# 0xC0000054/pdn-jpegxl

Hardware: AMD Instinct MI355X
Metric: megapixels/sec decode (4K lossy VarDCT) (higher is better)
Workload: dtype f32

## Files before the change

pdn_jpegxl_amd/csrc/dev_util.h:

```cpp
#pragma once
#include <stdint.h>
#include <hip/hip_fp16.h>

namespace jxlhip {

__host__ __device__ __forceinline__ int ReflectIndex(int v, int n) {
  while (v < 0 || v >= n) v = v < 0 ? -v - 1 : 2 * n - 1 - v;
  return v;
}

__device__ __forceinline__ uint32_t IntToOutSample(int32_t v, int bits, int out_bits) {
  const int32_t maxv = (int32_t)((1u << bits) - 1);
  if (bits == out_bits) return (uint32_t)min(maxv, max(0, v));
  float f = (float)v * (1.0f / (float)maxv);
  f *= out_bits == 16 ? 65535.0f : 255.0f;
  const float top = out_bits == 16 ? 65535.0f : 255.0f;
  if (!(f > 0.f)) return 0;
  if (f >= top) return (uint32_t)top;
  return (uint32_t)(f + 0.5f);
}

__device__ __forceinline__ float BitsToFloatSample(int32_t v, int bits) {
  if (bits == 32) return __int_as_float(v);
  return __half2float(__ushort_as_half((unsigned short)(v & 0xFFFF)));
}
__device__ __forceinline__ uint32_t FloatToOutBits(float f, int out_bits, int out_float) {
  if (out_float) return out_bits == 32 ? (uint32_t)__float_as_int(f) : (uint32_t)__half_as_ushort(__float2half_rn(f));
  const float top = out_bits == 16 ? 65535.0f : 255.0f;
  f *= top;
  if (!(f > 0.f)) return 0;
  if (f >= top) return (uint32_t)top;
  return (uint32_t)(f + 0.5f);
}
__device__ __forceinline__ uint32_t SampleToOutBits(int32_t v, int bits, int exp_bits, int out_bits, int out_float) {
  if (!out_float && !exp_bits) return IntToOutSample(v, bits, out_bits);
  const float f = exp_bits ? BitsToFloatSample(v, bits) : (float)v * (1.0f / (float)((1u << bits) - 1));
  return FloatToOutBits(f, out_bits, out_float);
}
__device__ __forceinline__ void StoreOutSample(uint8_t* base, size_t index, uint32_t raw, int out_bits) {
  if (out_bits == 8) base[index] = (uint8_t)raw;
  else if (out_bits == 16) ((uint16_t*)base)[index] = (uint16_t)raw;
  else ((uint32_t*)base)[index] = raw;
}

}
```

pdn_jpegxl_amd/csrc/entropy_kernels.hip:

```cpp
#include <hip/hip_runtime.h>
#include <cstdlib>
#include "dev_types.h"
#include "dev_util.h"
#include "kernels.h"

namespace jxlhip {

namespace {

__device__ const uint8_t d_order_bucket[kNumStrategies] = {0, 1, 1, 1, 2, 3, 4, 4, 5, 5, 6, 6, 1, 1, 1, 1, 1, 1, 7, 8, 8, 9, 10, 10, 11, 12, 12};
__device__ const uint8_t d_log2cx[kNumStrategies] = {0, 0, 0, 0, 1, 2, 0, 1, 0, 2, 1, 2, 0, 0, 0, 0, 0, 0, 3, 2, 3, 4, 3, 4, 5, 4, 5};
__device__ const uint8_t d_log2cy[kNumStrategies] = {0, 0, 0, 0, 1, 2, 1, 0, 2, 0, 2, 1, 0, 0, 0, 0, 0, 0, 3, 3, 2, 4, 4, 3, 5, 5, 4};
__device__ const uint8_t d_nnz_ctx[64] = {0,   0,   31,  62,  62,  93,  93,  93,  93,  123, 123, 123, 123, 152, 152, 152, 152, 152, 152, 152, 152, 180,
                                          180, 180, 180, 180, 180, 180, 180, 180, 180, 180, 180, 206, 206, 206, 206, 206, 206, 206, 206, 206, 206, 206,
                                          206, 206, 206, 206, 206, 206, 206, 206, 206, 206, 206, 206, 206, 206, 206, 206, 206, 206, 206, 206};

__device__ __forceinline__ int CeilLog2D(uint32_t x) { return x <= 1 ? 0 : 32 - __clz(x - 1); }
__device__ __forceinline__ int32_t UnpackSigned(uint32_t u) { return (int32_t)(u >> 1) ^ -(int32_t)(u & 1); }
#ifndef JXLHIP_PRIO_SERIAL
#define JXLHIP_PRIO_SERIAL 0
#endif
#if JXLHIP_PRIO_SERIAL
#define JXL_SERIAL_PRIO() __builtin_amdgcn_s_setprio(JXLHIP_PRIO_SERIAL)
#else
// ... 1147 lines not shown
          const int es = s_info[j];
          const int lcx = d_log2cx[es], lcy = d_log2cy[es], cx = 1 << lcx, cy = 1 << lcy;
          int wi = 0;
          uint32_t before = 0;
#pragma unroll
          for (int k = 1; k < 8; k++) { const bool past = pre[k] <= off; wi += past ? 1 : 0; before = past ? pre[k] : before; }
          uint32_t word = ~s_cov[y * 8 + wi];
          const int lim = min(32, bw - wi * 32);
          if (lim < 32) word &= (1u << lim) - 1;
          uint32_t rem = off - before;
          int xb = 0;
#pragma unroll
          for (int sft = 16; sft; sft >>= 1) {
            const uint32_t c = (uint32_t)__popc((word >> xb) & ((1u << sft) - 1));
            if (rem >= c) { rem -= c; xb += sft; }
          }
          const int x = wi * 32 + xb;
          const uint32_t mask = (cx == 32 ? 0xFFFFFFFFu : ((1u << cx) - 1)) << xb;
          if (off + (uint32_t)cx > nfree || x + cx > bw || y + cy > bh || xb + cx > 32 || (y & 31) + cy > 32 || (word & mask) != mask) {
            bad = true;
          } else {
            for (int iy = 1; iy < cy; iy++)
              if (atomicOr(&s_cov[(y + iy) * 8 + wi], mask) & mask) bad = true;
            s_pos[j] = x | y << 8;
          }
        }
      }
      const int n_row = __syncthreads_count(inrow);
      if (__syncthreads_or(bad || (nfree && !n_row))) { layout_bad = true; break; }
      num += (uint32_t)n_row;
    }
  }
  __threadfence_block();
  __syncthreads();
  if (s_flag || layout_bad || num != count) err |= kErrBlockLayout;
  if (tid == 0) s_count = (err & kErrBlockLayout) ? 0u : num;
  __syncthreads();
  const uint32_t placed = s_count;
  for (uint32_t i = tid; i < placed; i += 256) {
    const int x = s_pos[i] & 0xFF, y = s_pos[i] >> 8;
    const int s = s_info[i], q = 1 + s_info[count + i];
    const int lcx = d_log2cx[s], lcy = d_log2cy[s], cx = 1 << lcx, cy = 1 << lcy;
    const size_t cell = (size_t)(by0 + y) * im.w8 + bx0 + x;
    for (int iy = 0; iy < cy; iy++)
      for (int ix = 0; ix < cx; ix++) {
        const size_t cc = cell + (size_t)iy * im.w8 + ix;
        im.cellinfo[cc] = (uint32_t)s | ix << 8 | iy << 13 | lcx << 18 | lcy << 21 | 1u << 31;
        im.rawq[cc] = (uint16_t)q;
      }
  }
  if (err) SetError(im, err, 2, g);
}

__global__ __launch_bounds__(64) void hf_blocklist_kernel(const DevImage* __restrict__ imgs) {
  const DevImage& im = imgs[blockIdx.y];
  const int g = blockIdx.x;
  if (g >= im.ng || im.is_modular) return;
  const int lane = threadIdx.x;
  const int gx = g % im.xg, gy = g / im.xg;
  const int bx0 = gx * kGroupBlocks, by0 = gy * kGroupBlocks;
  const int bw = min(kGroupBlocks, im.w8 - bx0), bh = min(kGroupBlocks, im.h8 - by0);
  uint32_t* list = im.blk_list + (size_t)g * 1024;
  const int n_qf = im.n_qf;
  uint32_t total = 0;
  for (int it = 0; it < 16; it++) {
    const int idx = it * 64 + lane;
    const int bx = idx & 31, by = idx >> 5;
    bool first = false;
    uint32_t info = 0;
    if (bx < bw && by < bh) {
      info = im.cellinfo[(size_t)(by0 + by) * im.w8 + bx0 + bx];
      first = (info & 0x8003FF00u) == 0x80000000u;
    }
    const uint64_t m = __ballot(first);
    if (first) {
      const uint32_t pos = total + (uint32_t)__popcll(m & (((uint64_t)1 << lane) - 1));
      const uint32_t s = info & 0xFF, lcx = (info >> 18) & 7, lcy = (info >> 21) & 7;
      const uint32_t ord = d_order_bucket[s];
      const uint32_t rq = im.rawq[(size_t)(by0 + by) * im.w8 + bx0 + bx];
      uint32_t qf_idx = 0;
      for (int i = 0; i < n_qf; i++) qf_idx += rq > im.qf_thr[i];
      uint32_t lf_idx = 0;
      if (im.num_lf_ctx > 1) {
        const size_t cell = (size_t)(by0 + by) * im.w8 + bx0 + bx;
        uint32_t ix = 0, iy = 0, ib = 0;
        for (int i = 0; i < im.n_lf_thr[0]; i++) ix += im.lfq[0][cell] > im.lf_thr[0][i];
        for (int i = 0; i < im.n_lf_thr[1]; i++) iy += im.lfq[1][cell] > im.lf_thr[1][i];
        for (int i = 0; i < im.n_lf_thr[2]; i++) ib += im.lfq[2][cell] > im.lf_thr[2][i];
        lf_idx = (ix * (uint32_t)(im.n_lf_thr[2] + 1) + ib) * (uint32_t)(im.n_lf_thr[1] + 1) + iy;
      }
      uint32_t ctxs = 0;
      for (int ci = 0; ci < 3; ci++) {
        const int c = ci == 0 ? 1 : (ci == 1 ? 0 : 2);
        const uint32_t cprime = c < 2 ? (c ^ 1) : 2;
        ctxs |= ((uint32_t)im.block_ctx_map[((cprime * kNumOrders + ord) * (n_qf + 1) + qf_idx) * im.num_lf_ctx + lf_idx] & 31u) << (5 * ci);
      }
      list[pos] = (uint32_t)bx | (uint32_t)by << 5 | lcx << 10 | lcy << 13 | ctxs << 16;
    }
    total += (uint32_t)__popcll(m);
  }
  if (lane == 0) im.blk_count[g] = total;
}

template <bool kLds, int kRing>
__global__ __launch_bounds__(512) void hf_decode_kernel(const DevImage* imgs, const SectionTask* tasks, int lane_stride) {
  JXL_SERIAL_PRIO();
  constexpr int kTop = kRing / 2;
  constexpr int kQ = kRing / 4;
  typedef LaneBitsT<kRing, kRing / 4> Bits;
  extern __shared__ __align__(16) uint8_t smem[];
  const SectionTask task = tasks[blockIdx.x];
  const DevImage& im = imgs[task.image];
  const int per_wave = 64 / lane_stride;
  const int nslots = (task.count + 3) & ~3;
  CodeTab<kLds> tab;
  typename AS<kLds>::U8 nnz_tab;
  JXL_LDS uint8_t* nzcol;
  JXL_LDS uint32_t* ring_base;
  JXL_LDS uint32_t* descq;
  {
    JXL_LDS uint8_t* lds = (JXL_LDS uint8_t*)smem;
    size_t off = 0;
    ring_base = (JXL_LDS uint32_t*)lds; off += (size_t)nslots * kRing * 4;
    descq = (JXL_LDS uint32_t*)(lds + off); off += (size_t)nslots * 2 * kQ * 4;
    nzcol = lds + off; off += (size_t)nslots * 96;
    if constexpr (kLds) {
      off = StageCode(lds, off, im.acode, tab, threadIdx.x, blockDim.x);
      JXL_LDS uint8_t* sn = lds + off; off += 64;
      if (threadIdx.x < 64) sn[threadIdx.x] = d_nnz_ctx[threadIdx.x];
      nnz_tab = sn;
      __syncthreads();
    } else {
      GlobalCode(im.acode, tab);
      nnz_tab = d_nnz_ctx;
    }
  }
  if ((int)(threadIdx.x & 63) >= per_wave) return;
  const int si = (threadIdx.x >> 6) * per_wave + (threadIdx.x & 63);
  if (si >= task.count || si >= nslots) return;
  JXL_LDS uint8_t* const col = nzcol + si;
  const int g = im.hf_order[task.first + si];
  const int sec = im.single ? 0 : im.hf_sec_base + g;
  const uint64_t sec_bits = im.single ? im.hf_start_bits : im.sec_off[sec] * 8;
  Bits b;
  b.Init(im.cs, im.cs_size, sec_bits, ring_base + si, (uint32_t)nslots);
  const uint32_t preset = b.Read(CeilLog2D((uint32_t)im.num_presets));
  const uint32_t nbc = im.num_block_ctx;
  const uint32_t ctx_offset = preset * nbc * 495;
  uint32_t err = preset >= (uint32_t)im.num_presets ? (uint32_t)kErrBitstream : 0u;
  if (im.lz_hf) b.SetLz(im.lz_hf + ((size_t)g << 18), 18, 0);
  uint32_t state = InitAnsState(b, tab);
  const int gx = g % im.xg, gy = g / im.xg;
  const JXL_GLB uint32_t* const list = G(im.blk_list + (size_t)g * 1024);
  const uint32_t nblk = im.blk_count[g];
  JXL_LDS uint32_t* const dq = descq + si;
  constexpr uint32_t dqmask = 2u * kQ - 1;
  uint32_t bi = 0, dfilled = 0, it = 0, dpend_n = 0;
  uint32_t dpend[kQ];
#pragma unroll
  for (int i = 0; i < kQ; i++) dpend[i] = 0u;
  JXL_GLB uint32_t* const ent = G(im.centries) + (size_t)(g - im.centries_g0) * kGroupEntriesCap;
  const uint32_t ncells = (uint32_t)im.w8 * (uint32_t)im.h8;
  JXL_GLB U2* const cblk = (JXL_GLB U2*)G(im.cblk) + (size_t)(gy * kGroupBlocks) * im.w8 + (size_t)gx * kGroupBlocks;
  const uint32_t w8 = (uint32_t)im.w8;
  uint32_t epos = 0;
  uint32_t bx = 0, by = 0, lcx = 0, log2c = 0, covered = 1, size = 64, ctxs = 0, cell = 0;
  int ci = 3;
  uint32_t nzeros = 0, k = 0, prev = 0, histo = 0;
  bool want_nz = true;
#ifdef JXLHIP_PROFILE_HF
  const uint64_t pf_start = clock64();
  uint64_t pf_scalar = 0, pf_period = 0, pf_tokens = 0, pf_entries = 0, pf_periods = 0, pf_general = 0, pf_general_n = 0;
#endif
  uint32_t cfg_uni = 0;
  bool cfg_is_uni = false;
  if (per_wave == 1 && !tab.slow) {
    cfg_uni = tab.cfg[0] & 0xFFF;
    cfg_is_uni = true;
    for (uint32_t i = 1; i < tab.dc->num_clusters; i++) cfg_is_uni &= (tab.cfg[i] & 0xFFF) == cfg_uni;
    cfg_uni = (uint32_t)__builtin_amdgcn_readfirstlane((int)cfg_uni);
    cfg_is_uni = __builtin_amdgcn_readfirstlane((int)cfg_is_uni) != 0;
  }
  while (!err) {
    if ((it & (kTop - 1)) == 0) {
#ifdef JXLHIP_PROFILE_HF
      const uint64_t pf_t0 = clock64();
      pf_periods++;
#endif
      b.TopUp();
      if (dpend_n) {
#pragma unroll
        for (int i = 0; i < kQ; i++) if ((uint32_t)i < dpend_n) dq[__umul24((dfilled + i) & dqmask, nslots)] = dpend[i];
        dfilled += dpend_n;
        dpend_n = 0;
      }
      if (dfilled < min(nblk, bi + kQ)) {
        const uint32_t lim = min(nblk, bi + kQ);
        uint32_t v[kQ];
#pragma unroll
        for (int i = 0; i < kQ; i++) { v[i] = 0u; if (dfilled + i < lim) v[i] = list[dfilled + i]; }
#pragma unroll
        for (int i = 0; i < kQ; i++) if (dfilled + i < lim) dq[__umul24((dfilled + i) & dqmask, nslots)] = v[i];
        dfilled = lim;
      }
      {
        const uint32_t lim = min(nblk, bi + 2 * kQ);
        if (dfilled < lim) {
          dpend_n = min(lim - dfilled, (uint32_t)kQ);
#pragma unroll
          for (int i = 0; i < kQ; i++) { dpend[i] = 0u; if ((uint32_t)i < dpend_n) dpend[i] = list[dfilled + i]; }
        }
      }
#ifdef JXLHIP_PROFILE_HF
      pf_period += clock64() - pf_t0;
#endif
    }
    if (__all(!want_nz)) {
      if (per_wave == 1 && !tab.slow) {
#define JXL_RFL(x) ((uint32_t)__builtin_amdgcn_readfirstlane((int)(x)))
#ifdef JXLHIP_PROFILE_HF
        const uint64_t pf_t1 = clock64();
        pf_entries++;
#endif
        uint32_t s_state = JXL_RFL(state), s_nz = JXL_RFL(nzeros), s_k = JXL_RFL(k), s_prev = JXL_RFL(prev), s_epos = JXL_RFL(epos), s_it = JXL_RFL(it);
        const uint32_t s_cov = JXL_RFL(covered), s_l2 = JXL_RFL(log2c), s_size = JXL_RFL(size), s_histo = JXL_RFL(histo);
        uint64_t s_buf = ((uint64_t)JXL_RFL((uint32_t)(b.buf >> 32)) << 32) | JXL_RFL((uint32_t)b.buf);
        int s_n = (int)JXL_RFL(b.n);
        uint32_t s_rd = JXL_RFL(b.rd), s_rng = 0;
        const uint32_t la = JXL_RFL(tab.log_alpha), le = 12 - la;
        const uint32_t left = kTop - (s_it & (kTop - 1)), room = s_size > s_k ? s_size - s_k : 0u;
        const uint32_t cnt0 = min(left, room);
        uint32_t cnt = cnt0;
        uint32_t s_a = s_histo + 2 * JXL_RFL(nnz_tab[(s_nz + s_cov - 1) >> s_l2]);
        uint32_t s_cidx = 0xFFFFFFFFu, s_cl = 0;
        if (cnt) do {
          const uint32_t ks = s_k >> s_l2;
          const uint32_t fctx = min(ks - 1, min(7 + (ks >> 1), 15 + (ks >> 2)));
          const uint32_t cidx = s_a + fctx * 2 + s_prev;
          if (cidx != s_cidx) { s_cl = JXL_RFL(tab.cmap[cidx]); s_cidx = cidx; }
          const uint32_t cl = s_cl;
          const uint32_t res = s_state & 0xFFF, i = res >> le, pos = res & ((1u << le) - 1);
          const uint64_t e = tab.alias[(cl << la) | i];
          uint32_t c = cfg_uni;
          if (__builtin_expect(!cfg_is_uni, 0)) c = JXL_RFL(tab.cfg[cl]);
          const uint32_t x = JXL_RFL((uint32_t)e), y = JXL_RFL((uint32_t)(e >> 32));
          const bool gt = pos >= (x & 0xFF);
          const uint32_t sym = gt ? ((x >> 8) & 0xFF) : i;
          const uint32_t off = gt ? (y & 0xFFFF) + pos : pos;
          const uint32_t freq = gt ? ((x >> 16) ^ (y >> 16)) : (x >> 16);
          s_state = freq * (s_state >> 12) + off;
          if (s_state < 65536u) {
            if (s_n <= 32) { s_buf |= (uint64_t)JXL_RFL(b.ring[__umul24(s_rd & (kRing - 1), b.rs)]) << s_n; s_n += 32; s_rd++; }
            s_state = (s_state << 16) | ((uint32_t)s_buf & 0xFFFFu);
            s_buf >>= 16; s_n -= 16;
          }
          uint32_t u = sym;
          const uint32_t se = c & 0xF, split = 1u << se;
          if (__builtin_expect(sym >= split, 0)) {
            const uint32_t msb = (c >> 4) & 0xF, lsb = (c >> 8) & 0xF;
            const uint32_t nb = se - (msb + lsb) + ((sym - split) >> (msb + lsb)), nbr = nb > 32 ? 32 : nb;
            if (s_n <= 32) { s_buf |= (uint64_t)JXL_RFL(b.ring[__umul24(s_rd & (kRing - 1), b.rs)]) << s_n; s_n += 32; s_rd++; }
            const uint32_t bits = (uint32_t)(s_buf & (((uint64_t)1 << nbr) - 1));
            s_buf >>= nbr; s_n -= (int)nbr;
            const uint32_t low = sym & ((1u << lsb) - 1), hi = (1u << msb) | ((sym >> lsb) & ((1u << msb) - 1));
            u = (uint32_t)(((((uint64_t)hi << (nb & 63)) | bits) << lsb) | low);
          }
          cnt--;
          s_prev = 0;
          if (u) {
            const int32_t v = UnpackSigned(u);
            s_rng |= (uint32_t)(v + 0x8000);
            ent[s_epos++] = s_k | (uint32_t)v << 16;
            s_prev = 1;
            s_k++;
            if (--s_nz == 0) break;
            s_a = s_histo + 2 * JXL_RFL(nnz_tab[(s_nz + s_cov - 1) >> s_l2]);
          } else {
            s_k++;
          }
        } while (cnt);
        s_it += cnt0 - cnt;
#ifdef JXLHIP_PROFILE_HF
        pf_scalar += clock64() - pf_t1;
        pf_tokens += cnt0 - cnt;
#endif
        uint32_t s_err = s_rng > 0xFFFFu ? (uint32_t)kErrRange : 0u;
        if (s_nz != 0 && s_k >= s_size) s_err |= kErrBitstream;
#undef JXL_RFL
        state = s_state; nzeros = s_nz; k = s_k; prev = s_prev; epos = s_epos; it = s_it;
        b.buf = s_buf; b.n = s_n; b.rd = s_rd;
        err |= s_err;
        if (s_nz == 0 && !s_err) { want_nz = true; ci++; }
        continue;
      }
      for (;;) {
        const uint32_t nzl = (nzeros + covered - 1) >> log2c;
        const uint32_t ks = k >> log2c;
        const uint32_t fctx = ks < 16 ? ks - 1 : (ks < 32 ? 15 + ((ks - 16) >> 1) : 23 + ((ks - 32) >> 2));
        const uint32_t u = AnsGet(b, state, tab, histo + ((uint32_t)nnz_tab[nzl] + fctx) * 2 + prev);
        it++;
        bool leave = false;
        if (u) {
          const int32_t v = UnpackSigned(u);
          if (v != (int32_t)(int16_t)v) err |= kErrRange;
          ent[epos++] = k | (uint32_t)v << 16;
          prev = 1;
          if (--nzeros == 0) { want_nz = true; ci++; leave = true; }
        } else {
          prev = 0;
        }
        if (++k >= size && nzeros != 0) { err |= kErrBitstream; leave = true; }
        if (__any(leave) || (it & (kTop - 1)) == 0) break;
      }
      continue;
    }
#ifdef JXLHIP_PROFILE_HF
    const uint64_t pf_t2 = clock64();
    pf_general_n++;
#endif
    if (want_nz && ci >= 3) {
      if (bi >= nblk) break;
      const uint32_t d = dq[__umul24(bi & dqmask, nslots)];
      bi++;
      bx = d & 31; by = (d >> 5) & 31;
      lcx = (d >> 10) & 7;
      const uint32_t lcy = (d >> 13) & 7;
      ctxs = d >> 16;
      log2c = lcx + lcy; covered = 1u << log2c; size = covered << 6;
      cell = __umul24(by, w8) + bx;
      ci = 0;
    }
    const int c = ci == 0 ? 1 : (ci == 1 ? 0 : 2);
    uint32_t ctx;
    if (want_nz) {
      JXL_LDS uint8_t* const cc = col + __umul24(c * 32, nslots);
      uint32_t predicted;
      if (bx == 0) predicted = by == 0 ? 32u : (uint32_t)cc[0];
      else if (by == 0) predicted = cc[__umul24(bx - 1, nslots)];
      else predicted = ((uint32_t)cc[__umul24(bx, nslots)] + cc[__umul24(bx - 1, nslots)] + 1) >> 1;
      const uint32_t block_ctx = (ctxs >> (5 * ci)) & 31;
      uint32_t nzc = predicted >= 64 ? 64 : predicted;
      nzc = nzc < 8 ? nzc : 4 + nzc / 2;
      ctx = ctx_offset + nzc * nbc + block_ctx;
    } else {
      const uint32_t nzl = (nzeros + covered - 1) >> log2c;
      const uint32_t ks = k >> log2c;
      const uint32_t fctx = ks < 16 ? ks - 1 : (ks < 32 ? 15 + ((ks - 16) >> 1) : 23 + ((ks - 32) >> 2));
      ctx = histo + ((uint32_t)nnz_tab[nzl] + fctx) * 2 + prev;
    }
    const uint32_t u = AnsGet(b, state, tab, ctx);
    it++;
    if (want_nz) {
      nzeros = u;
      if (nzeros + covered > size) { err |= kErrBitstream; break; }
      const uint8_t fill = (uint8_t)((nzeros + covered - 1) >> log2c);
      JXL_LDS uint8_t* const cc = col + __umul24(c * 32 + bx, nslots);
      for (uint32_t ix = 0; ix < (1u << lcx); ix++) cc[__umul24(ix, nslots)] = fill;
      U2 rec;
      rec.x = epos; rec.y = nzeros;
      cblk[(size_t)c * ncells + cell] = rec;
      if (nzeros) {
        const uint32_t block_ctx = (ctxs >> (5 * ci)) & 31;
        histo = ctx_offset + nbc * 37 + 458 * block_ctx;
        prev = nzeros > size / 16 ? 0 : 1;
        k = covered;
        want_nz = false;
      } else {
        ci++;
      }
    } else {
      if (u) {
        const int32_t v = UnpackSigned(u);
        if (v != (int32_t)(int16_t)v) err |= kErrRange;
        ent[epos++] = k | (uint32_t)v << 16;
        prev = 1;
        if (--nzeros == 0) { want_nz = true; ci++; }
      } else {
        prev = 0;
      }
      if (++k >= size && nzeros != 0) { err |= kErrBitstream; break; }
    }
#ifdef JXLHIP_PROFILE_HF
    pf_general += clock64() - pf_t2;
#endif
  }
  if (!err && (state != 0x130000u || b.slow_err)) err |= kErrBitstream;
  const uint64_t used = b.Consumed();
  if (!err && sec_bits + used > (im.sec_off[sec] + im.sec_size[sec]) * 8) err |= kErrBitstream;
  im.grp_bitpos[g] = err ? ~(uint64_t)0 : sec_bits + used;
#ifdef JXLHIP_PROFILE_HF
  if (per_wave == 1)
    printf("[hfprof] g %d total %llu scalar-loop %llu (%llu entries, %llu tokens) period %llu (%llu periods) blocks %u general %llu (%llu iterations)\n", g,
           (unsigned long long)(clock64() - pf_start), (unsigned long long)pf_scalar, (unsigned long long)pf_entries,
           (unsigned long long)pf_tokens, (unsigned long long)pf_period, (unsigned long long)pf_periods, nblk,
           (unsigned long long)pf_general, (unsigned long long)pf_general_n);
#endif
  if (err) SetError(im, err, 3, g);
}

template <bool kLds, bool kGeneric = true>
__global__ __launch_bounds__(64) void alpha_ans_kernel(const DevImage* imgs, const SectionTask* tasks, int lane_stride, int scalar_rows) {
  JXL_SERIAL_PRIO();
  extern __shared__ __align__(16) uint8_t smem[];
  const SectionTask task = tasks[blockIdx.x];
  const DevImage& im = imgs[task.image];
  if (!im.has_alpha || im.alpha_in_global) return;
  ModTables<kLds> mt;
  const int slots = 64 / lane_stride;
  LoadModTables<kLds>(im, smem, (size_t)slots * kRingWords * 4, mt, threadIdx.x, 64, slots == 1 && scalar_rows);
  const int lane = threadIdx.x;
  if (lane >= slots || lane >= task.count) return;
  const int g = task.first + lane;
  ChanDesc* desc = im.alpha_desc + g;
  const uint64_t start = im.alpha_bitpos[g];
  if (start == ~(uint64_t)0) {
    ChanDesc d;
    d.kind = kChanFinal; d.value = 0; d.pad0 = 0; d.pad1 = 0;
    *desc = d;
    return;
  }
  const int gx = g % im.xg, gy = g / im.xg;
  const int sec = im.alpha_sec_base + g;
  LaneBits b;
  b.Init(im.cs, im.cs_size, start, (JXL_LDS uint32_t*)smem + lane, (uint32_t)slots);
  uint32_t err = 0;
  if (b.Read(4) != 3) err |= kErrUnsupportedHeader;
  else {
    const int x0 = gx * kGroupDim, y0 = gy * kGroupDim;
    const int gw = min(kGroupDim, im.w - x0), gh = min(kGroupDim, im.h - y0);
    if (im.lz_grp) b.SetLz(im.lz_grp + ((size_t)g << 16), 16, (uint32_t)gw);
    uint32_t state = InitAnsState(b, mt.tab);
    const int sid = 1 + 3 * im.nlf + kNumQuantTables + g;
    DecodeChannelLane<kLds, false, kGeneric>(b, state, mt.tab, mt.tree, 0, sid, gw, gh, im.alpha32 + (size_t)y0 * im.w + x0, im.w, desc,
                            im.wp_grp ? im.wp_grp + (size_t)g * im.wp_grp_ints : nullptr);
    if (state != 0x130000u || b.slow_err) err |= kErrBitstream;
    if (start + b.Consumed() > (im.sec_off[sec] + im.sec_size[sec]) * 8) err |= kErrBitstream;
  }
  if (err) {
    ChanDesc d;
    d.kind = kChanFinal; d.value = 0; d.pad0 = 0; d.pad1 = 0;
    *desc = d;
    SetError(im, err, 4, g);
  }
}

__device__ __forceinline__ int32_t RowRotateFromBelow(int32_t v) {
  return __builtin_amdgcn_update_dpp(0, v, 0x121 , 0xF, 0xF, false);
}
__device__ __forceinline__ bool AlphaRowsAreGradient(const I4* tree, int sid, int gh, int li, int nlanes) {
  bool ok = true;
  for (int r = li; r < gh; r += nlanes) { bool u = false; ok = ok && (RowNode(tree, 0, sid, r, &u).a & 0xFF) == 5; }
  return ok;
}
__device__ __forceinline__ bool AlphaGroupStatic(const DevImage& im, int g, int* gw, int* gh, int* sid, ChanDesc* d) {
  if (!im.has_alpha || im.is_modular || g < 0 || g >= im.ng || im.out_bits != 8 || im.alpha_bits != 8 || im.alpha_exp || (im.w & 3) != 0) return false;
  const int gx = g % im.xg, gy = g / im.xg;
  if (gy * kGroupDim >= im.band_y1 || (gy + 1) * kGroupDim <= im.band_y0) return false;
  *gw = min(kGroupDim, im.w - gx * kGroupDim); *gh = min(kGroupDim, im.h - gy * kGroupDim);
  *sid = im.alpha_in_global ? 0 : 1 + 3 * im.nlf + kNumQuantTables + g;
  *d = im.alpha_desc[g];
  return d->kind == kChanResid && (*gw & 15) == 0;
}
__global__ __launch_bounds__(64) void alpha_finish_gradient_kernel(const DevImage* __restrict__ imgs) {
  const DevImage& im = imgs[blockIdx.y];
  const int lane = threadIdx.x, sub = lane >> 4, li = lane & 15;
  const int g = blockIdx.x * 4 + sub;
  int gw = 0, gh = 0, sid = 0;
  ChanDesc d;
  d.kind = kChanFinal;
  bool mine = AlphaGroupStatic(im, g, &gw, &gh, &sid, &d);
  if (mine) mine = AlphaRowsAreGradient((const I4*)im.tree, sid, gh, li, 16);
  {
    const uint64_t bal = __ballot(mine);
    mine = ((bal >> (sub * 16)) & 0xFFFFu) == 0xFFFFu;
  }
  if (__ballot(mine) == 0) return;
  const int gx = mine ? g % im.xg : 0, gy = mine ? g / im.xg : 0;
  const int x0 = gx * kGroupDim, y0 = gy * kGroupDim;
  const int nq = mine ? gw >> 4 : 0, rows = mine ? gh : 0;
  const JXL_GLB int32_t* const plane = G(im.alpha32) + (size_t)y0 * im.w + x0;
  JXL_GLB uint8_t* const out = G(im.alpha) + (size_t)y0 * im.w + x0;
  int steps = rows + 15;
  steps = max(steps, __shfl_xor(steps, 16)); steps = max(steps, __shfl_xor(steps, 32));
  typedef int32_t __attribute__((ext_vector_type(4))) I4v;
  auto line_of = [&](int T, int* r_out, int* q_out) {
    const int m = T - li;
    const int r = (m >> 4) * 16 + li, q = m & 15;
    *r_out = r; *q_out = q;
    return m >= 0 && r < rows && q < nq;
  };
  auto load_line = [&](int T, I4v* v) {
    int r, q;
    const bool act = line_of(T, &r, &q);
    const int rc = act ? r : 0, qc = act ? q : 0;
    const JXL_GLB I4v* p = (const JXL_GLB I4v*)(plane + (size_t)(mine ? rc : 0) * im.w + qc * 16);
    v[0] = p[0]; v[1] = p[1]; v[2] = p[2]; v[3] = p[3];
  };
  if (mine && li == 0) im.alpha_desc[g].pad0 = 1;
  I4v cur[4], nxt[4];
  load_line(0, nxt);
  int32_t prev_out[16];
#pragma unroll
  for (int j = 0; j < 16; j++) prev_out[j] = 0;
  int32_t W = 0, n_last = 0;
  for (int T = 0; T < steps; T++) {
#pragma unroll
    for (int k = 0; k < 4; k++) cur[k] = nxt[k];
    load_line(T + 1, nxt);
    int r, q;
    const bool act = line_of(T, &r, &q);
    int32_t nq16[16];
#pragma unroll
    for (int j = 0; j < 16; j++) nq16[j] = RowRotateFromBelow(prev_out[j]);
    const bool top = r == 0;
    int32_t o[16];
#pragma unroll
    for (int j = 0; j < 16; j++) {
      const int32_t res = cur[j >> 2][j & 3];
      int32_t n, nw;
      if (top) { n = W; nw = W; }
      else { n = nq16[j]; nw = j == 0 ? n_last : nq16[j - 1]; }
      if (j == 0 && q == 0) {
        const int32_t w0 = top ? 0 : nq16[0];
        W = w0; n = w0; nw = w0;
      }
      const int32_t val = (int32_t)((uint32_t)res + (uint32_t)ClampedGradient32(W, n, nw));
      o[j] = val;
      W = val;
    }
    n_last = nq16[15];
    if (act) {
#pragma unroll
      for (int j = 0; j < 16; j++) prev_out[j] = o[j];
      uint32_t pk[4];
#pragma unroll
      for (int k = 0; k < 4; k++) {
        uint32_t wd = 0;
// ... 416 lines not shown
```

pdn_jpegxl_amd/csrc/selftest.cc:

```cpp
#include <hip/hip_runtime.h>
#include <cstring>
#include <stdexcept>
#include <string>
#include <vector>
#include "../../include/jxlfiletypeio.h"
#include "dev_util.h"
#include "enc_types.h"
#include "host_parse.h"
#include "host_write.h"
#include "icc.h"

namespace jxlhip {
std::vector<EncTreeNode> MakeEncoderTree(uint32_t nlf);
}
using namespace jxlhip;

static void SetEncErr(ErrorInfo* e, const char* msg) {
  if (!e || !msg) return;
  size_t n = strlen(msg);
  if (n == 0) return;
  if (n > 255) n = 255;
  memcpy(e->errorMessage, msg, n);
  e->errorMessage[n] = 0;
}

namespace jxlhip {
bool ReadBackTokens(const uint8_t* bytes, size_t nbytes, size_t num_ctx, const uint32_t* ctxs, const uint32_t* values, size_t n, std::string* why);
bool ReadBackTree(const uint8_t* bytes, size_t nbytes, std::vector<DevTreeNode>* tree, std::string* why);
}

extern "C" JXLFILETYPEIO_API int32_t jxlhip_selftest_entropy(uint32_t seed, uint32_t num_ctx, uint32_t n, int32_t max_clusters,
                                                             uint32_t pinned_ctx_plus1, ErrorInfo* err) {
  try {
    uint64_t s = seed * 0x9E3779B97F4A7C15ull + 12345;
    auto rnd = [&]() { s ^= s << 13; s ^= s >> 7; s ^= s << 17; return (uint32_t)(s >> 32); };
    std::vector<uint32_t> ctxs(n), vals(n), hist((size_t)num_ctx * kEncAlphabet, 0);
    std::vector<uint8_t> pinned(num_ctx, 0);
    if (pinned_ctx_plus1) pinned[pinned_ctx_plus1 - 1] = 1;
    for (uint32_t i = 0; i < n; i++) {
      const uint32_t c = rnd() % num_ctx;
      uint32_t v = 0;
      const uint32_t spread = 1 + c % 7;
      while ((rnd() % (spread + 1)) != 0 && v < 40) v++;
      if (rnd() % 97 == 0) v = rnd() >> (rnd() % 30);
      if (pinned[c]) v = 0;
      ctxs[i] = c; vals[i] = v;
      uint32_t tok, nb, bits;
      HybridEncode(v, &tok, &nb, &bits);
      hist[(size_t)c * kEncAlphabet + tok]++;
    }
    BitWriter bw;
    EncCode code;
    BuildAndWriteCode(hist.data(), num_ctx, max_clusters, pinned, bw, code);
    std::vector<EncToken> toks;
    for (uint32_t i = 0; i < n; i++)
      if (!pinned[ctxs[i]]) toks.push_back(EncToken{ctxs[i], vals[i]});
    WriteTokensHost(toks, code, bw);
    std::vector<uint8_t> bytes = bw.Finish();
    std::string why;
    if (!ReadBackTokens(bytes.data(), bytes.size(), num_ctx, ctxs.data(), vals.data(), n, &why)) { SetEncErr(err, why.c_str()); return 1; }
    return 0;
  } catch (const std::exception& e) {
    SetEncErr(err, e.what());
    return 2;
  }
}

extern "C" JXLFILETYPEIO_API int32_t jxlhip_selftest_tree(uint32_t nlf, ErrorInfo* err) {
  try {
    const std::vector<EncTreeNode> t = MakeEncoderTree(nlf);
    BitWriter bw;
    WriteTree(t, bw);
    std::vector<uint8_t> bytes = bw.Finish();
    std::vector<DevTreeNode> back;
    std::string why;
    if (!ReadBackTree(bytes.data(), bytes.size(), &back, &why)) { SetEncErr(err, why.c_str()); return 1; }
    if (back.size() != t.size()) { SetEncErr(err, "node count"); return 2; }
    uint32_t leaf = 0;
    for (size_t i = 0; i < t.size(); i++) {
      if (t[i].property >= 0) {
        if (back[i].property != t[i].property || back[i].splitval != t[i].splitval) { SetEncErr(err, "inner node"); return 3; }
      } else {
        if (back[i].property >= 0 || (back[i].a & 0xFF) != (uint32_t)t[i].pred || (back[i].a >> 8) != leaf || back[i].splitval != t[i].offset ||
            back[i].b != t[i].multiplier) { SetEncErr(err, "leaf"); return 4; }
        leaf++;
      }
    }
    return leaf == kNumEncLeaves ? 0 : 5;
  } catch (const std::exception& e) {
    SetEncErr(err, e.what());
    return 6;
  }
}

extern "C" JXLFILETYPEIO_API size_t jxlhip_selftest_headers(uint32_t xsize, uint32_t ysize, int32_t gray, int32_t alpha, int32_t lossless,
                                                            uint32_t epf_iters, uint32_t sec_bytes, uint8_t* dst, size_t capacity) {
  try {
    EncImageInfo ii;
    ii.xsize = xsize; ii.ysize = ysize; ii.gray = gray != 0; ii.alpha = alpha != 0; ii.xyb = !lossless;
    EncFrameInfo fi;
    fi.encoding = lossless ? 1 : 0;
    fi.gab = !lossless; fi.epf_iters = lossless ? 0 : epf_iters;
    BitWriter cs;
    WriteCodestreamHeaders(ii, cs);
    WriteFrameHeader(ii, fi, cs);
    const uint32_t ng = ((xsize + 255) / 256) * ((ysize + 255) / 256), nlf = ((xsize + 2047) / 2048) * ((ysize + 2047) / 2048);
    std::vector<uint32_t> sizes(ng == 1 ? 1 : 2 + nlf + ng, sec_bytes);
    WriteToc(sizes, cs);
    std::vector<uint8_t> bytes = cs.Finish();
    bytes.resize(bytes.size() + (size_t)sec_bytes * sizes.size(), 0);
    std::vector<uint8_t> file = WriteContainer(bytes, nullptr, 0, nullptr, 0);
    if (file.size() > capacity) return 0;
    memcpy(dst, file.data(), file.size());
    return file.size();
  } catch (...) {
    return 0;
  }
}

extern "C" JXLFILETYPEIO_API size_t jxlhip_selftest_headers_icc(uint32_t xsize, uint32_t ysize, int32_t alpha, int32_t lossless, const uint8_t* icc,
                                                                size_t icc_size, uint8_t* dst, size_t capacity) {
  try {
    EncImageInfo ii;
    ii.xsize = xsize; ii.ysize = ysize; ii.gray = false; ii.alpha = alpha != 0; ii.xyb = !lossless;
    ii.icc = icc; ii.icc_size = icc_size;
    EncFrameInfo fi;
    fi.encoding = lossless ? 1 : 0;
    fi.gab = !lossless; fi.epf_iters = lossless ? 0 : 1;
    BitWriter cs;
    WriteCodestreamHeaders(ii, cs);
    WriteFrameHeader(ii, fi, cs);
    const uint32_t ng = ((xsize + 255) / 256) * ((ysize + 255) / 256), nlf = ((xsize + 2047) / 2048) * ((ysize + 2047) / 2048);
    std::vector<uint32_t> sizes(ng == 1 ? 1 : 2 + nlf + ng, 3);
    WriteToc(sizes, cs);
    std::vector<uint8_t> bytes = cs.Finish();
    bytes.resize(bytes.size() + 3 * sizes.size(), 0);
    std::vector<uint8_t> file = WriteContainer(bytes, nullptr, 0, nullptr, 0);
    if (file.size() > capacity) return 0;
    memcpy(dst, file.data(), file.size());
    return file.size();
  } catch (...) {
    return 0;
  }
}

extern "C" JXLFILETYPEIO_API int32_t jxlhip_selftest_reflect(int32_t v, int32_t n) { return ReflectIndex(v, n); }
```

Before: 29780.

## Add dedicated multi-slot-per-wave HF coefficient decode loop with look-ahead neighbor prefetch

Splits the HF coefficient decode into a separate loop for the per_wave>1 non-slow case. That loop prefetches the next block descriptor and its top/left nonzero-count neighbors from LDS one block ahead, and computes all three channels' nonzero contexts at block start. It also replaces the nnz_tab lookup with an arithmetic bucket function, and unifies the nonzero-count and coefficient token paths into a single AnsGet per iteration, which cuts divergence. The aim is to hide LDS/descriptor latency and shorten the serial dependency chain between tokens, at the cost of more registers and a duplicated code path. An empty asm barrier on nblk forces it into a VGPR.

```diff
diff --git a/pdn_jpegxl_amd/csrc/dev_util.h b/pdn_jpegxl_amd/csrc/dev_util.h
--- a/pdn_jpegxl_amd/csrc/dev_util.h
+++ b/pdn_jpegxl_amd/csrc/dev_util.h
@@ -7,6 +7,11 @@
 __host__ __device__ __forceinline__ int ReflectIndex(int v, int n) {
   while (v < 0 || v >= n) v = v < 0 ? -v - 1 : 2 * n - 1 - v;
   return v;
+}
+
+__host__ __device__ __forceinline__ uint32_t NnzBucketCtx(uint32_t nzl) {
+  const uint32_t b = (nzl >= 2) + (nzl >= 3) + (nzl >= 5) + (nzl >= 9) + (nzl >= 13) + (nzl >= 21) + (nzl >= 33);
+  return (uint32_t)(0xCEB4987B5D3E1F00ull >> (8 * b)) & 0xFFu;
 }
 
 __device__ __forceinline__ uint32_t IntToOutSample(int32_t v, int bits, int out_bits) {
diff --git a/pdn_jpegxl_amd/csrc/entropy_kernels.hip b/pdn_jpegxl_amd/csrc/entropy_kernels.hip
--- a/pdn_jpegxl_amd/csrc/entropy_kernels.hip
+++ b/pdn_jpegxl_amd/csrc/entropy_kernels.hip
@@ -1323,7 +1323,8 @@
   uint32_t state = InitAnsState(b, tab);
   const int gx = g % im.xg, gy = g / im.xg;
   const JXL_GLB uint32_t* const list = G(im.blk_list + (size_t)g * 1024);
-  const uint32_t nblk = im.blk_count[g];
+  uint32_t nblk = im.blk_count[g];
+  asm volatile("" : "+v"(nblk));
   JXL_LDS uint32_t* const dq = descq + si;
   constexpr uint32_t dqmask = 2u * kQ - 1;
   uint32_t bi = 0, dfilled = 0, it = 0, dpend_n = 0;
@@ -1352,208 +1353,298 @@
     cfg_uni = (uint32_t)__builtin_amdgcn_readfirstlane((int)cfg_uni);
     cfg_is_uni = __builtin_amdgcn_readfirstlane((int)cfg_is_uni) != 0;
   }
-  while (!err) {
-    if ((it & (kTop - 1)) == 0) {
+  uint32_t nz_ctx0 = 0, nz_ctx1 = 0, nz_ctx2 = 0;
+  uint32_t d_next = 0, d_after = 0;
+  uint32_t up0 = 0, up1 = 0, up2 = 0, lf0 = 0, lf1 = 0, lf2 = 0;
+  uint32_t pbx = 0, pcx = 0, fv0 = 0, fv1 = 0, fv2 = 0;
+  auto period = [&]() {
 #ifdef JXLHIP_PROFILE_HF
-      const uint64_t pf_t0 = clock64();
-      pf_periods++;
+    const uint64_t pf_t0 = clock64();
+    pf_periods++;
 #endif
-      b.TopUp();
-      if (dpend_n) {
+    b.TopUp();
+    if (dpend_n) {
 #pragma unroll
-        for (int i = 0; i < kQ; i++) if ((uint32_t)i < dpend_n) dq[__umul24((dfilled + i) & dqmask, nslots)] = dpend[i];
-        dfilled += dpend_n;
-        dpend_n = 0;
-      }
-      if (dfilled < min(nblk, bi + kQ)) {
-        const uint32_t lim = min(nblk, bi + kQ);
-        uint32_t v[kQ];
+      for (int i = 0; i < kQ; i++) if ((uint32_t)i < dpend_n) dq[__umul24((dfilled + i) & dqmask, nslots)] = dpend[i];
+      dfilled += dpend_n;
+      dpend_n = 0;
+    }
+    if (dfilled < min(nblk, bi + kQ)) {
+      const uint32_t lim = min(nblk, bi + kQ);
+      uint32_t v[kQ];
 #pragma unroll
-        for (int i = 0; i < kQ; i++) { v[i] = 0u; if (dfilled + i < lim) v[i] = list[dfilled + i]; }
+      for (int i = 0; i < kQ; i++) { v[i] = 0u; if (dfilled + i < lim) v[i] = list[dfilled + i]; }
 #pragma unroll
-        for (int i = 0; i < kQ; i++) if (dfilled + i < lim) dq[__umul24((dfilled + i) & dqmask, nslots)] = v[i];
-        dfilled = lim;
-      }
-      {
-        const uint32_t lim = min(nblk, bi + 2 * kQ);
-        if (dfilled < lim) {
-          dpend_n = min(lim - dfilled, (uint32_t)kQ);
+      for (int i = 0; i < kQ; i++) if (dfilled + i < lim) dq[__umul24((dfilled + i) & dqmask, nslots)] = v[i];
+      dfilled = lim;
+    }
+    {
+      const uint32_t lim = min(nblk, bi + 2 * kQ);
+      if (dfilled < lim) {
+        dpend_n = min(lim - dfilled, (uint32_t)kQ);
 #pragma unroll
-          for (int i = 0; i < kQ; i++) { dpend[i] = 0u; if ((uint32_t)i < dpend_n) dpend[i] = list[dfilled + i]; }
+        for (int i = 0; i < kQ; i++) { dpend[i] = 0u; if ((uint32_t)i < dpend_n) dpend[i] = list[dfilled + i]; }
+      }
+    }
+#ifdef JXLHIP_PROFILE_HF
+    pf_period += clock64() - pf_t0;
+#endif
+  };
+  if (per_wave > 1 && !tab.slow) {
+    while (!err) {
+      if ((it & (kTop - 1)) == 0) period();
+      auto colv = [&](uint32_t c, uint32_t x) { return (uint32_t)col[__umul24(c * 32 + x, nslots)]; };
+      auto look_ahead = [&]() {
+        const uint32_t x = d_next & 31, xl = x ? x - 1 : 0;
+        up0 = colv(1, x); lf0 = colv(1, xl);
+        up1 = colv(0, x); lf1 = colv(0, xl);
+        up2 = colv(2, x); lf2 = colv(2, xl);
+      };
+      if (want_nz && ci >= 3) {
+        if (bi >= nblk) break;
+        if (bi == 0) {
+          d_next = dq[0];
+          d_after = dq[__umul24(1u & dqmask, nslots)];
+          look_ahead();
+          pcx = 0;
         }
-      }
-#ifdef JXLHIP_PROFILE_HF
-      pf_period += clock64() - pf_t0;
-#endif
-    }
-    if (__all(!want_nz)) {
-      if (per_wave == 1 && !tab.slow) {
-#define JXL_RFL(x) ((uint32_t)__builtin_amdgcn_readfirstlane((int)(x)))
-#ifdef JXLHIP_PROFILE_HF
-        const uint64_t pf_t1 = clock64();
-        pf_entries++;
-#endif
-        uint32_t s_state = JXL_RFL(state), s_nz = JXL_RFL(nzeros), s_k = JXL_RFL(k), s_prev = JXL_RFL(prev), s_epos = JXL_RFL(epos), s_it = JXL_RFL(it);
-        const uint32_t s_cov = JXL_RFL(covered), s_l2 = JXL_RFL(log2c), s_size = JXL_RFL(size), s_histo = JXL_RFL(histo);
-        uint64_t s_buf = ((uint64_t)JXL_RFL((uint32_t)(b.buf >> 32)) << 32) | JXL_RFL((uint32_t)b.buf);
-        int s_n = (int)JXL_RFL(b.n);
-        uint32_t s_rd = JXL_RFL(b.rd), s_rng = 0;
-        const uint32_t la = JXL_RFL(tab.log_alpha), le = 12 - la;
-        const uint32_t left = kTop - (s_it & (kTop - 1)), room = s_size > s_k ? s_size - s_k : 0u;
-        const uint32_t cnt0 = min(left, room);
-        uint32_t cnt = cnt0;
-        uint32_t s_a = s_histo + 2 * JXL_RFL(nnz_tab[(s_nz + s_cov - 1) >> s_l2]);
-        uint32_t s_cidx = 0xFFFFFFFFu, s_cl = 0;
-        if (cnt) do {
-          const uint32_t ks = s_k >> s_l2;
-          const uint32_t fctx = min(ks - 1, min(7 + (ks >> 1), 15 + (ks >> 2)));
-          const uint32_t cidx = s_a + fctx * 2 + s_prev;
-          if (cidx != s_cidx) { s_cl = JXL_RFL(tab.cmap[cidx]); s_cidx = cidx; }
-          const uint32_t cl = s_cl;
-          const uint32_t res = s_state & 0xFFF, i = res >> le, pos = res & ((1u << le) - 1);
-          const uint64_t e = tab.alias[(cl << la) | i];
-          uint32_t c = cfg_uni;
-          if (__builtin_expect(!cfg_is_uni, 0)) c = JXL_RFL(tab.cfg[cl]);
-          const uint32_t x = JXL_RFL((uint32_t)e), y = JXL_RFL((uint32_t)(e >> 32));
-          const bool gt = pos >= (x & 0xFF);
-          const uint32_t sym = gt ? ((x >> 8) & 0xFF) : i;
-          const uint32_t off = gt ? (y & 0xFFFF) + pos : pos;
-          const uint32_t freq = gt ? ((x >> 16) ^ (y >> 16)) : (x >> 16);
-          s_state = freq * (s_state >> 12) + off;
-          if (s_state < 65536u) {
-            if (s_n <= 32) { s_buf |= (uint64_t)JXL_RFL(b.ring[__umul24(s_rd & (kRing - 1), b.rs)]) << s_n; s_n += 32; s_rd++; }
-            s_state = (s_state << 16) | ((uint32_t)s_buf & 0xFFFFu);
-            s_buf >>= 16; s_n -= 16;
-          }
-          uint32_t u = sym;
-          const uint32_t se = c & 0xF, split = 1u << se;
-          if (__builtin_expect(sym >= split, 0)) {
-            const uint32_t msb = (c >> 4) & 0xF, lsb = (c >> 8) & 0xF;
-            const uint32_t nb = se - (msb + lsb) + ((sym - split) >> (msb + lsb)), nbr = nb > 32 ? 32 : nb;
-            if (s_n <= 32) { s_buf |= (uint64_t)JXL_RFL(b.ring[__umul24(s_rd & (kRing - 1), b.rs)]) << s_n; s_n += 32; s_rd++; }
-            const uint32_t bits = (uint32_t)(s_buf & (((uint64_t)1 << nbr) - 1));
-            s_buf >>= nbr; s_n -= (int)nbr;
-            const uint32_t low = sym & ((1u << lsb) - 1), hi = (1u << msb) | ((sym >> lsb) & ((1u << msb) - 1));
-            u = (uint32_t)(((((uint64_t)hi << (nb & 63)) | bits) << lsb) | low);
-          }
-          cnt--;
-          s_prev = 0;
-          if (u) {
-            const int32_t v = UnpackSigned(u);
-            s_rng |= (uint32_t)(v + 0x8000);
-            ent[s_epos++] = s_k | (uint32_t)v << 16;
-            s_prev = 1;
-            s_k++;
-            if (--s_nz == 0) break;
-            s_a = s_histo + 2 * JXL_RFL(nnz_tab[(s_nz + s_cov - 1) >> s_l2]);
-          } else {
-            s_k++;
-          }
-        } while (cnt);
-        s_it += cnt0 - cnt;
-#ifdef JXLHIP_PROFILE_HF
-        pf_scalar += clock64() - pf_t1;
-        pf_tokens += cnt0 - cnt;
-#endif
-        uint32_t s_err = s_rng > 0xFFFFu ? (uint32_t)kErrRange : 0u;
-        if (s_nz != 0 && s_k >= s_size) s_err |= kErrBitstream;
-#undef JXL_RFL
-        state = s_state; nzeros = s_nz; k = s_k; prev = s_prev; epos = s_epos; it = s_it;
-        b.buf = s_buf; b.n = s_n; b.rd = s_rd;
-        err |= s_err;
-        if (s_nz == 0 && !s_err) { want_nz = true; ci++; }
-        continue;
-      }
-      for (;;) {
-        const uint32_t nzl = (nzeros + covered - 1) >> log2c;
-        const uint32_t ks = k >> log2c;
-        const uint32_t fctx = ks < 16 ? ks - 1 : (ks < 32 ? 15 + ((ks - 16) >> 1) : 23 + ((ks - 32) >> 2));
-        const uint32_t u = AnsGet(b, state, tab, histo + ((uint32_t)nnz_tab[nzl] + fctx) * 2 + prev);
-        it++;
-        bool leave = false;
+        const uint32_t d = d_next;
+        bx = d & 31; by = (d >> 5) & 31;
+        lcx = (d >> 10) & 7;
+        const uint32_t lcy = (d >> 13) & 7;
+        ctxs = d >> 16;
+        log2c = lcx + lcy; covered = 1u << log2c; size = covered << 6;
+        cell = __umul24(by, w8) + bx;
+        ci = 0;
+        const uint32_t xl = bx ? bx - 1 : 0;
+        const bool up_prev = bx - pbx < pcx, lf_prev = xl - pbx < pcx;
+        auto nz_ctx = [&](uint32_t up, uint32_t lf, uint32_t fv, uint32_t block_ctx) {
+          const uint32_t a = up_prev ? fv : up, l = lf_prev ? fv : lf;
+          uint32_t p = bx == 0 ? (by == 0 ? 32u : a) : (by == 0 ? l : (a + l + 1) >> 1);
+          p = p >= 64 ? 64 : p;
+          p = p < 8 ? p : 4 + p / 2;
+          return ctx_offset + p * nbc + block_ctx;
+        };
+        nz_ctx0 = nz_ctx(up0, lf0, fv0, ctxs & 31);
+        nz_ctx1 = nz_ctx(up1, lf1, fv1, (ctxs >> 5) & 31);
+        nz_ctx2 = nz_ctx(up2, lf2, fv2, (ctxs >> 10) & 31);
+        pbx = bx; pcx = 1u << lcx;
+        bi++;
+        d_next = d_after;
+        look_ahead();
+        d_after = dq[__umul24((bi + 1) & dqmask, nslots)];
+      }
+      const uint32_t nzl = (nzeros + covered - 1) >> log2c;
+      const uint32_t ks = k >> log2c;
+      const uint32_t fctx = min(ks - 1, min(7 + (ks >> 1), 15 + (ks >> 2)));
+      const uint32_t nzc = ci == 0 ? nz_ctx0 : (ci == 1 ? nz_ctx1 : nz_ctx2);
+      const uint32_t u = AnsGet(b, state, tab, want_nz ? nzc : histo + (NnzBucketCtx(nzl) + fctx) * 2 + prev);
+      it++;
+      if (want_nz) {
+        nzeros = u;
+        if (nzeros + covered > size) { err |= kErrBitstream; break; }
+        const uint32_t fill = (nzeros + covered - 1) >> log2c;
+        const int c = ci == 0 ? 1 : (ci == 1 ? 0 : 2);
+        JXL_LDS uint8_t* const cc = col + __umul24(c * 32 + bx, nslots);
+        for (uint32_t ix = 0; ix < (1u << lcx); ix++) cc[__umul24(ix, nslots)] = (uint8_t)fill;
+        fv0 = ci == 0 ? fill : fv0; fv1 = ci == 1 ? fill : fv1; fv2 = ci == 2 ? fill : fv2;
+        U2 rec;
+        rec.x = epos; rec.y = nzeros;
+        cblk[(size_t)c * ncells + cell] = rec;
+        if (nzeros) {
+          const uint32_t block_ctx = (ctxs >> (5 * ci)) & 31;
+          histo = ctx_offset + nbc * 37 + 458 * block_ctx;
+          prev = nzeros > size / 16 ? 0 : 1;
+          k = covered;
+          want_nz = false;
+        } else {
+          ci++;
+        }
+      } else {
         if (u) {
           const int32_t v = UnpackSigned(u);
           if (v != (int32_t)(int16_t)v) err |= kErrRange;
           ent[epos++] = k | (uint32_t)v << 16;
           prev = 1;
-          if (--nzeros == 0) { want_nz = true; ci++; leave = true; }
+          if (--nzeros == 0) { want_nz = true; ci++; }
         } else {
           prev = 0;
         }
-        if (++k >= size && nzeros != 0) { err |= kErrBitstream; leave = true; }
-        if (__any(leave) || (it & (kTop - 1)) == 0) break;
-      }
-      continue;
-    }
-#ifdef JXLHIP_PROFILE_HF
-    const uint64_t pf_t2 = clock64();
-    pf_general_n++;
-#endif
-    if (want_nz && ci >= 3) {
-      if (bi >= nblk) break;
-      const uint32_t d = dq[__umul24(bi & dqmask, nslots)];
-      bi++;
-      bx = d & 31; by = (d >> 5) & 31;
-      lcx = (d >> 10) & 7;
-      const uint32_t lcy = (d >> 13) & 7;
-      ctxs = d >> 16;
-      log2c = lcx + lcy; covered = 1u << log2c; size = covered << 6;
-      cell = __umul24(by, w8) + bx;
-      ci = 0;
-    }
-    const int c = ci == 0 ? 1 : (ci == 1 ? 0 : 2);
-    uint32_t ctx;
-    if (want_nz) {
-      JXL_LDS uint8_t* const cc = col + __umul24(c * 32, nslots);
-      uint32_t predicted;
-      if (bx == 0) predicted = by == 0 ? 32u : (uint32_t)cc[0];
-      else if (by == 0) predicted = cc[__umul24(bx - 1, nslots)];
-      else predicted = ((uint32_t)cc[__umul24(bx, nslots)] + cc[__umul24(bx - 1, nslots)] + 1) >> 1;
-      const uint32_t block_ctx = (ctxs >> (5 * ci)) & 31;
-      uint32_t nzc = predicted >= 64 ? 64 : predicted;
-      nzc = nzc < 8 ? nzc : 4 + nzc / 2;
-      ctx = ctx_offset + nzc * nbc + block_ctx;
-    } else {
-      const uint32_t nzl = (nzeros + covered - 1) >> log2c;
-      const uint32_t ks = k >> log2c;
-      const uint32_t fctx = ks < 16 ? ks - 1 : (ks < 32 ? 15 + ((ks - 16) >> 1) : 23 + ((ks - 32) >> 2));
-      ctx = histo + ((uint32_t)nnz_tab[nzl] + fctx) * 2 + prev;
-    }
-    const uint32_t u = AnsGet(b, state, tab, ctx);
-    it++;
-    if (want_nz) {
-      nzeros = u;
-      if (nzeros + covered > size) { err |= kErrBitstream; break; }
-      const uint8_t fill = (uint8_t)((nzeros + covered - 1) >> log2c);
-      JXL_LDS uint8_t* const cc = col + __umul24(c * 32 + bx, nslots);
-      for (uint32_t ix = 0; ix < (1u << lcx); ix++) cc[__umul24(ix, nslots)] = fill;
-      U2 rec;
-      rec.x = epos; rec.y = nzeros;
-      cblk[(size_t)c * ncells + cell] = rec;
-      if (nzeros) {
+        if (++k >= size && nzeros != 0) { err |= kErrBitstream; break; }
+      }
+    }
+  } else {
+    while (!err) {
+      if ((it & (kTop - 1)) == 0) period();
+      if (__all(!want_nz)) {
+        if (per_wave == 1 && !tab.slow) {
+  #define JXL_RFL(x) ((uint32_t)__builtin_amdgcn_readfirstlane((int)(x)))
+  #ifdef JXLHIP_PROFILE_HF
+          const uint64_t pf_t1 = clock64();
+          pf_entries++;
+  #endif
+          uint32_t s_state = JXL_RFL(state), s_nz = JXL_RFL(nzeros), s_k = JXL_RFL(k), s_prev = JXL_RFL(prev), s_epos = JXL_RFL(epos), s_it = JXL_RFL(it);
+          const uint32_t s_cov = JXL_RFL(covered), s_l2 = JXL_RFL(log2c), s_size = JXL_RFL(size), s_histo = JXL_RFL(histo);
+          uint64_t s_buf = ((uint64_t)JXL_RFL((uint32_t)(b.buf >> 32)) << 32) | JXL_RFL((uint32_t)b.buf);
+          int s_n = (int)JXL_RFL(b.n);
+          uint32_t s_rd = JXL_RFL(b.rd), s_rng = 0;
+          const uint32_t la = JXL_RFL(tab.log_alpha), le = 12 - la;
+          const uint32_t left = kTop - (s_it & (kTop - 1)), room = s_size > s_k ? s_size - s_k : 0u;
+          const uint32_t cnt0 = min(left, room);
+          uint32_t cnt = cnt0;
+          uint32_t s_a = s_histo + 2 * JXL_RFL(nnz_tab[(s_nz + s_cov - 1) >> s_l2]);
+          uint32_t s_cidx = 0xFFFFFFFFu, s_cl = 0;
+          if (cnt) do {
+            const uint32_t ks = s_k >> s_l2;
+            const uint32_t fctx = min(ks - 1, min(7 + (ks >> 1), 15 + (ks >> 2)));
+            const uint32_t cidx = s_a + fctx * 2 + s_prev;
+            if (cidx != s_cidx) { s_cl = JXL_RFL(tab.cmap[cidx]); s_cidx = cidx; }
+            const uint32_t cl = s_cl;
+            const uint32_t res = s_state & 0xFFF, i = res >> le, pos = res & ((1u << le) - 1);
+            const uint64_t e = tab.alias[(cl << la) | i];
+            uint32_t c = cfg_uni;
+            if (__builtin_expect(!cfg_is_uni, 0)) c = JXL_RFL(tab.cfg[cl]);
+            const uint32_t x = JXL_RFL((uint32_t)e), y = JXL_RFL((uint32_t)(e >> 32));
+            const bool gt = pos >= (x & 0xFF);
+            const uint32_t sym = gt ? ((x >> 8) & 0xFF) : i;
+            const uint32_t off = gt ? (y & 0xFFFF) + pos : pos;
+            const uint32_t freq = gt ? ((x >> 16) ^ (y >> 16)) : (x >> 16);
+            s_state = freq * (s_state >> 12) + off;
+            if (s_state < 65536u) {
+              if (s_n <= 32) { s_buf |= (uint64_t)JXL_RFL(b.ring[__umul24(s_rd & (kRing - 1), b.rs)]) << s_n; s_n += 32; s_rd++; }
+              s_state = (s_state << 16) | ((uint32_t)s_buf & 0xFFFFu);
+              s_buf >>= 16; s_n -= 16;
+            }
+            uint32_t u = sym;
+            const uint32_t se = c & 0xF, split = 1u << se;
+            if (__builtin_expect(sym >= split, 0)) {
+              const uint32_t msb = (c >> 4) & 0xF, lsb = (c >> 8) & 0xF;
+              const uint32_t nb = se - (msb + lsb) + ((sym - split) >> (msb + lsb)), nbr = nb > 32 ? 32 : nb;
+              if (s_n <= 32) { s_buf |= (uint64_t)JXL_RFL(b.ring[__umul24(s_rd & (kRing - 1), b.rs)]) << s_n; s_n += 32; s_rd++; }
+              const uint32_t bits = (uint32_t)(s_buf & (((uint64_t)1 << nbr) - 1));
+              s_buf >>= nbr; s_n -= (int)nbr;
+              const uint32_t low = sym & ((1u << lsb) - 1), hi = (1u << msb) | ((sym >> lsb) & ((1u << msb) - 1));
+              u = (uint32_t)(((((uint64_t)hi << (nb & 63)) | bits) << lsb) | low);
+            }
+            cnt--;
+            s_prev = 0;
+            if (u) {
+              const int32_t v = UnpackSigned(u);
+              s_rng |= (uint32_t)(v + 0x8000);
+              ent[s_epos++] = s_k | (uint32_t)v << 16;
+              s_prev = 1;
+              s_k++;
+              if (--s_nz == 0) break;
+              s_a = s_histo + 2 * JXL_RFL(nnz_tab[(s_nz + s_cov - 1) >> s_l2]);
+            } else {
+              s_k++;
+            }
+          } while (cnt);
+          s_it += cnt0 - cnt;
+  #ifdef JXLHIP_PROFILE_HF
+          pf_scalar += clock64() - pf_t1;
+          pf_tokens += cnt0 - cnt;
+  #endif
+          uint32_t s_err = s_rng > 0xFFFFu ? (uint32_t)kErrRange : 0u;
+          if (s_nz != 0 && s_k >= s_size) s_err |= kErrBitstream;
+  #undef JXL_RFL
+          state = s_state; nzeros = s_nz; k = s_k; prev = s_prev; epos = s_epos; it = s_it;
+          b.buf = s_buf; b.n = s_n; b.rd = s_rd;
+          err |= s_err;
+          if (s_nz == 0 && !s_err) { want_nz = true; ci++; }
+          continue;
+        }
+        for (;;) {
+          const uint32_t nzl = (nzeros + covered - 1) >> log2c;
+          const uint32_t ks = k >> log2c;
+          const uint32_t fctx = ks < 16 ? ks - 1 : (ks < 32 ? 15 + ((ks - 16) >> 1) : 23 + ((ks - 32) >> 2));
+          const uint32_t u = AnsGet(b, state, tab, histo + ((uint32_t)nnz_tab[nzl] + fctx) * 2 + prev);
+          it++;
+          bool leave = false;
+          if (u) {
+            const int32_t v = UnpackSigned(u);
+            if (v != (int32_t)(int16_t)v) err |= kErrRange;
+            ent[epos++] = k | (uint32_t)v << 16;
+            prev = 1;
+            if (--nzeros == 0) { want_nz = true; ci++; leave = true; }
+          } else {
+            prev = 0;
+          }
+          if (++k >= size && nzeros != 0) { err |= kErrBitstream; leave = true; }
+          if (__any(leave) || (it & (kTop - 1)) == 0) break;
+        }
+        continue;
+      }
+  #ifdef JXLHIP_PROFILE_HF
+      const uint64_t pf_t2 = clock64();
+      pf_general_n++;
+  #endif
+      if (want_nz && ci >= 3) {
+        if (bi >= nblk) break;
+        const uint32_t d = dq[__umul24(bi & dqmask, nslots)];
+        bi++;
+        bx = d & 31; by = (d >> 5) & 31;
+        lcx = (d >> 10) & 7;
+        const uint32_t lcy = (d >> 13) & 7;
+        ctxs = d >> 16;
+        log2c = lcx + lcy; covered = 1u << log2c; size = covered << 6;
+        cell = __umul24(by, w8) + bx;
+        ci = 0;
+      }
+      const int c = ci == 0 ? 1 : (ci == 1 ? 0 : 2);
+      uint32_t ctx;
+      if (want_nz) {
+        JXL_LDS uint8_t* const cc = col + __umul24(c * 32, nslots);
+        uint32_t predicted;
+        if (bx == 0) predicted = by == 0 ? 32u : (uint32_t)cc[0];
+        else if (by == 0) predicted = cc[__umul24(bx - 1, nslots)];
+        else predicted = ((uint32_t)cc[__umul24(bx, nslots)] + cc[__umul24(bx - 1, nslots)] + 1) >> 1;
         const uint32_t block_ctx = (ctxs >> (5 * ci)) & 31;
-        histo = ctx_offset + nbc * 37 + 458 * block_ctx;
-        prev = nzeros > size / 16 ? 0 : 1;
-        k = covered;
-        want_nz = false;
+        uint32_t nzc = predicted >= 64 ? 64 : predicted;
+        nzc = nzc < 8 ? nzc : 4 + nzc / 2;
+        ctx = ctx_offset + nzc * nbc + block_ctx;
       } else {
-        ci++;
-      }
-    } else {
-      if (u) {
-        const int32_t v = UnpackSigned(u);
-        if (v != (int32_t)(int16_t)v) err |= kErrRange;
-        ent[epos++] = k | (uint32_t)v << 16;
-        prev = 1;
-        if (--nzeros == 0) { want_nz = true; ci++; }
+        const uint32_t nzl = (nzeros + covered - 1) >> log2c;
+        const uint32_t ks = k >> log2c;
+        const uint32_t fctx = ks < 16 ? ks - 1 : (ks < 32 ? 15 + ((ks - 16) >> 1) : 23 + ((ks - 32) >> 2));
+        ctx = histo + ((uint32_t)nnz_tab[nzl] + fctx) * 2 + prev;
+      }
+      const uint32_t u = AnsGet(b, state, tab, ctx);
+      it++;
+      if (want_nz) {
+        nzeros = u;
+        if (nzeros + covered > size) { err |= kErrBitstream; break; }
+        const uint8_t fill = (uint8_t)((nzeros + covered - 1) >> log2c);
+        JXL_LDS uint8_t* const cc = col + __umul24(c * 32 + bx, nslots);
+        for (uint32_t ix = 0; ix < (1u << lcx); ix++) cc[__umul24(ix, nslots)] = fill;
+        U2 rec;
+        rec.x = epos; rec.y = nzeros;
+        cblk[(size_t)c * ncells + cell] = rec;
+        if (nzeros) {
+          const uint32_t block_ctx = (ctxs >> (5 * ci)) & 31;
+          histo = ctx_offset + nbc * 37 + 458 * block_ctx;
+          prev = nzeros > size / 16 ? 0 : 1;
+          k = covered;
+          want_nz = false;
+        } else {
+          ci++;
+        }
       } else {
-        prev = 0;
-      }
-      if (++k >= size && nzeros != 0) { err |= kErrBitstream; break; }
-    }
-#ifdef JXLHIP_PROFILE_HF
-    pf_general += clock64() - pf_t2;
-#endif
+        if (u) {
+          const int32_t v = UnpackSigned(u);
+          if (v != (int32_t)(int16_t)v) err |= kErrRange;
+          ent[epos++] = k | (uint32_t)v << 16;
+          prev = 1;
+          if (--nzeros == 0) { want_nz = true; ci++; }
+        } else {
+          prev = 0;
+        }
+        if (++k >= size && nzeros != 0) { err |= kErrBitstream; break; }
+      }
+  #ifdef JXLHIP_PROFILE_HF
+      pf_general += clock64() - pf_t2;
+  #endif
+    }
   }
   if (!err && (state != 0x130000u || b.slow_err)) err |= kErrBitstream;
   const uint64_t used = b.Consumed();
diff --git a/pdn_jpegxl_amd/csrc/selftest.cc b/pdn_jpegxl_amd/csrc/selftest.cc
--- a/pdn_jpegxl_amd/csrc/selftest.cc
+++ b/pdn_jpegxl_amd/csrc/selftest.cc
@@ -145,3 +145,5 @@
 }
 
 extern "C" JXLFILETYPEIO_API int32_t jxlhip_selftest_reflect(int32_t v, int32_t n) { return ReflectIndex(v, n); }
+
+extern "C" JXLFILETYPEIO_API uint32_t jxlhip_selftest_nnz_ctx(uint32_t nzl) { return NnzBucketCtx(nzl); }
```

New measurement: 30380, median of 6. 1.02x the previous value.
